# WangChangqi98/CSS

Hardware: NVIDIA B200
Metric: contrastive_path_pixels_per_sec (higher is better)
Workload: dtype f32

## Files before the change

### css_b200/csrc/css_grad.cu

```cuda
#include "css_common.cuh"

#define GSL_ELEMS 8192
#define GSL_THREADS 256
#define GSL_BATCH 24
#define GSL_PF_ANCH 3
#define GSL_LIST_MAX 6144

__device__ __forceinline__ void slab_apply(float* __restrict__ slab, const float* __restrict__ grad_anchor, float go, int a, int s, int hw,
                                           int r0, int q0, int m0, int q1, int m1) {
    const int d_min = q0 + (s < m0), d_max = q1 - (s > m1);
    const float* ga = grad_anchor + (size_t)a * CSS_D;
    for (int d = d_min; d <= d_max; d += 4) {
        float g[4];
#pragma unroll
        for (int u = 0; u < 4; ++u) g[u] = (d + u <= d_max) ? __ldg(ga + d + u) : 0.f;
#pragma unroll
        for (int u = 0; u < 4; ++u)
            if (d + u <= d_max) atomicAdd(&slab[(d + u) * hw + s - r0], go * g[u]);
    }
}

__global__ void __launch_bounds__(GSL_THREADS, 4) grad_slab_kernel(const float* __restrict__ grad_out, const int32_t* __restrict__ anchor_px,
                                                                   const float* __restrict__ grad_anchor, int n_anchor, int hw,
                                                                   int list_cap, float* __restrict__ grad_rep) {
    css_pdl_enter();
    extern __shared__ __align__(16) float slab[];
    __shared__ int s_cnt;
    int* list_a = reinterpret_cast<int*>(slab + GSL_ELEMS);
    int* list_s = list_a + list_cap;
    const int b = blockIdx.y;
    const int img = CSS_D * hw;
    const int px_lo = b * hw, px_hi = px_lo + hw;
    if (threadIdx.x == 0) s_cnt = 0;
    __syncthreads();
    for (int a0 = 0; a0 < n_anchor; a0 += GSL_THREADS * GSL_BATCH) {
        int px[GSL_BATCH];
#pragma unroll
        for (int i = 0; i < GSL_BATCH; ++i) {
            const int a = a0 + i * GSL_THREADS + threadIdx.x;
            px[i] = a < n_anchor ? __ldg(anchor_px + a) : -1;
        }
#pragma unroll
        for (int i = 0; i < GSL_BATCH; ++i) {
            if (px[i] >= px_lo && px[i] < px_hi) {
                const int pos = atomicAdd(&s_cnt, 1);
                if (pos < list_cap) {
                    list_a[pos] = a0 + i * GSL_THREADS + threadIdx.x;
                    list_s[pos] = px[i] - px_lo;
                }
            }
        }
    }
    __syncthreads();
    const int cnt = s_cnt;
    const float go = __ldg(grad_out);
    float4* slab4 = reinterpret_cast<float4*>(slab);
    float* out_img = grad_rep + (size_t)b * img;
    const int n_slabs = (img + GSL_ELEMS - 1) / GSL_ELEMS;
    for (int i = threadIdx.x; i < GSL_ELEMS / 4; i += GSL_THREADS) slab4[i] = make_float4(0.f, 0.f, 0.f, 0.f);
    __syncthreads();
    if (cnt <= GSL_THREADS * GSL_PF_ANCH && cnt <= list_cap && 2 * hw >= GSL_ELEMS) {
        float pv[GSL_PF_ANCH][2];
        int po[GSL_PF_ANCH][2];
        auto gather = [&](int j) {
            const int r0 = j * GSL_ELEMS, r1 = min(r0 + GSL_ELEMS, img);
            const int q0 = r0 / hw, m0 = r0 - q0 * hw, q1 = (r1 - 1) / hw, m1 = (r1 - 1) - q1 * hw;
#pragma unroll
            for (int u = 0; u < GSL_PF_ANCH; ++u) {
                const int t = threadIdx.x + u * GSL_THREADS;
                po[u][0] = po[u][1] = -1;
                if (t < cnt) {
                    const int a = list_a[t], sp = list_s[t];
                    const int d_min = q0 + (sp < m0), d_max = q1 - (sp > m1);
                    const float* ga = grad_anchor + (size_t)a * CSS_D;
#pragma unroll
                    for (int c = 0; c < 2; ++c) {
                        if (d_min + c <= d_max) {
                            pv[u][c] = __ldg(ga + d_min + c);
                            po[u][c] = (d_min + c) * hw + sp - r0;
                        }
                    }
                }
            }
        };
        int j = blockIdx.x;
        if (j < n_slabs) gather(j);
        for (; j < n_slabs; j += gridDim.x) {
#pragma unroll
            for (int u = 0; u < GSL_PF_ANCH; ++u)
#pragma unroll
                for (int c = 0; c < 2; ++c)
                    if (po[u][c] >= 0) atomicAdd(&slab[po[u][c]], go * pv[u][c]);
            __syncthreads();
            const int r0 = j * GSL_ELEMS, r1 = min(r0 + GSL_ELEMS, img);
            if (j + (int)gridDim.x < n_slabs) gather(j + gridDim.x);
            float4* out4 = reinterpret_cast<float4*>(out_img + r0);
            const int n4 = (r1 - r0) >> 2;
            for (int i = threadIdx.x; i < GSL_ELEMS / 4; i += GSL_THREADS) {
                if (i < n4) __stcs(out4 + i, slab4[i]);
                slab4[i] = make_float4(0.f, 0.f, 0.f, 0.f);
            }
            __syncthreads();
        }
        return;
    }
    for (int j = blockIdx.x; j < n_slabs; j += gridDim.x) {
        const int r0 = j * GSL_ELEMS, r1 = min(r0 + GSL_ELEMS, img);
        const int q0 = r0 / hw, m0 = r0 - q0 * hw, q1 = (r1 - 1) / hw, m1 = (r1 - 1) - q1 * hw;
        if (cnt <= list_cap) {
            for (int t = threadIdx.x; t < cnt; t += GSL_THREADS) slab_apply(slab, grad_anchor, go, list_a[t], list_s[t], hw, r0, q0, m0, q1, m1);
        } else {
            for (int a = threadIdx.x; a < n_anchor; a += GSL_THREADS) {
                const int px = __ldg(anchor_px + a);
                if (px >= px_lo && px < px_hi) slab_apply(slab, grad_anchor, go, a, px - px_lo, hw, r0, q0, m0, q1, m1);
            }
        }
        __syncthreads();
        float4* out4 = reinterpret_cast<float4*>(out_img + r0);
        const int n4 = (r1 - r0) >> 2;
        for (int i = threadIdx.x; i < GSL_ELEMS / 4; i += GSL_THREADS) {
            if (i < n4) __stcs(out4 + i, slab4[i]);
            slab4[i] = make_float4(0.f, 0.f, 0.f, 0.f);
        }
        __syncthreads();
    }
}

#define GS_PER_BLOCK 8
__global__ void __launch_bounds__(CSS_D) grad_scatter_kernel(const float* __restrict__ grad_out, const int32_t* __restrict__ anchor_px,
                                                             const float* __restrict__ grad_anchor, int n_anchor, int hw,
                                                             float* __restrict__ grad_rep) {
    css_pdl_enter();
    const int base = blockIdx.x * GS_PER_BLOCK;
    int px[GS_PER_BLOCK];
    float g[GS_PER_BLOCK];
#pragma unroll
    for (int i = 0; i < GS_PER_BLOCK; ++i) px[i] = (base + i < n_anchor) ? __ldg(anchor_px + base + i) : -1;
    const float go = __ldg(grad_out);
#pragma unroll
    for (int i = 0; i < GS_PER_BLOCK; ++i)
        g[i] = (px[i] >= 0) ? ldg_stream(grad_anchor + (size_t)(base + i) * CSS_D + threadIdx.x) : 0.f;
#pragma unroll
    for (int i = 0; i < GS_PER_BLOCK; ++i) {
        if (px[i] < 0) continue;
        const int b = px[i] / hw, s = px[i] - b * hw;
        atomicAdd(grad_rep + ((size_t)b * CSS_D + threadIdx.x) * hw + s, go * g[i]);
    }
}

#define GSL_MAX_ANCHORS 32768

extern "C" int css_grad_scatter(const float* grad_out, const int32_t* anchor_px, const float* grad_anchor, int n_anchor, int B2,
                                int D, int h, int w, float* grad_rep, void* stream) {
    CSS_CHECK_ARG(grad_out && anchor_px && grad_anchor && grad_rep, CSS_E_ARG, "css_grad_scatter: null pointer");
    CSS_CHECK_ARG(n_anchor > 0 && B2 > 0 && h > 0 && w > 0, CSS_E_ARG, "css_grad_scatter: non-positive size");
    CSS_CHECK_ARG(D == CSS_D, CSS_E_DIM, "css_grad_scatter: D must be %d", CSS_D);
    cudaStream_t st = (cudaStream_t)stream;
    const long long total = (long long)B2 * D * h * w;
    if (n_anchor <= GSL_MAX_ANCHORS && ((uintptr_t)grad_rep & 15) == 0 && B2 <= 65535 && (long long)D * h * w < (1ll << 30)) {
        int list_cap = 4 * ((n_anchor + B2 - 1) / B2);
        if (list_cap < 1024) list_cap = 1024;
        if (list_cap > n_anchor) list_cap = n_anchor;
        if (list_cap > GSL_LIST_MAX) list_cap = GSL_LIST_MAX;
        const int smem = GSL_ELEMS * (int)sizeof(float) + 2 * list_cap * (int)sizeof(int);
        cudaError_t e = cudaFuncSetAttribute(grad_slab_kernel, cudaFuncAttributeMaxDynamicSharedMemorySize, smem);
        if (e != cudaSuccess) { css_set_error("css_grad_scatter: cudaFuncSetAttribute: %s", cudaGetErrorString(e)); return (int)e; }
        const int n_slabs = (int)(((long long)D * h * w + GSL_ELEMS - 1) / GSL_ELEMS);
        int per_sm = (227 * 1024) / (smem + 1024);
        if (per_sm > 4) per_sm = 4;
        int G = per_sm * css_sm_count() / B2;
        if (G > n_slabs) G = n_slabs;
        if (G < 1) G = 1;
        css_launch(grad_slab_kernel, dim3(dim3(G, B2)), dim3(GSL_THREADS), (size_t)(smem), (cudaStream_t)(st), grad_out, anchor_px, grad_anchor, n_anchor, h * w, list_cap, grad_rep);
        CSS_CHECK_LAUNCH("css_grad_scatter", 1);
        return 0;
    }
    cudaError_t e = cudaMemsetAsync(grad_rep, 0, sizeof(float) * (size_t)total, st);
    if (e != cudaSuccess) { css_set_error("css_grad_scatter: memset: %s", cudaGetErrorString(e)); return (int)e; }
    css_launch(grad_scatter_kernel, dim3((n_anchor + GS_PER_BLOCK - 1) / GS_PER_BLOCK), dim3(CSS_D), (size_t)(0), (cudaStream_t)(st), grad_out, anchor_px, grad_anchor, n_anchor, h * w,
                                                                                      grad_rep);
    CSS_CHECK_LAUNCH("css_grad_scatter", 1);
    return 0;
}


__global__ void __launch_bounds__(CSS_D) grad_rows_kernel(const float* __restrict__ grad_out, const int32_t* __restrict__ anchor_px,
                                                          const float* __restrict__ grad_anchor, int n_anchor, float* __restrict__ grad_rows) {
    css_pdl_enter();
    const int base = blockIdx.x * GS_PER_BLOCK;
    int px[GS_PER_BLOCK];
    float g[GS_PER_BLOCK];
#pragma unroll
    for (int i = 0; i < GS_PER_BLOCK; ++i) px[i] = (base + i < n_anchor) ? __ldg(anchor_px + base + i) : -1;
    const float go = __ldg(grad_out);
#pragma unroll
    for (int i = 0; i < GS_PER_BLOCK; ++i)
        g[i] = (px[i] >= 0) ? ldg_stream(grad_anchor + (size_t)(base + i) * CSS_D + threadIdx.x) : 0.f;
#pragma unroll
    for (int i = 0; i < GS_PER_BLOCK; ++i)
        if (px[i] >= 0) atomicAdd(grad_rows + (size_t)px[i] * CSS_D + threadIdx.x, go * g[i]);
}

extern "C" int css_grad_scatter_nhwc(const float* grad_out, const int32_t* anchor_px, const float* grad_anchor, int n_anchor, int B2, int D,
                                     int h, int w, float* grad_rows, void* stream) {
    CSS_CHECK_ARG(grad_out && anchor_px && grad_anchor && grad_rows, CSS_E_ARG, "css_grad_scatter_nhwc: null pointer");
    CSS_CHECK_ARG(n_anchor > 0 && B2 > 0 && h > 0 && w > 0, CSS_E_ARG, "css_grad_scatter_nhwc: non-positive size");
    CSS_CHECK_ARG(D == CSS_D, CSS_E_DIM, "css_grad_scatter_nhwc: D must be %d", CSS_D);
    cudaStream_t st = (cudaStream_t)stream;
    cudaError_t e = cudaMemsetAsync(grad_rows, 0, sizeof(float) * (size_t)B2 * D * h * w, st);
    if (e != cudaSuccess) { css_set_error("css_grad_scatter_nhwc: memset: %s", cudaGetErrorString(e)); return (int)e; }
    css_launch(grad_rows_kernel, dim3((n_anchor + GS_PER_BLOCK - 1) / GS_PER_BLOCK), dim3(CSS_D), (size_t)0, st, grad_out, anchor_px, grad_anchor, n_anchor,
               grad_rows);
    CSS_CHECK_LAUNCH("css_grad_scatter_nhwc", 1);
    return 0;
}
```

Measured before the change: 228.0 million.

## Double-buffer slab and write out with TMA bulk async stores

The slab accumulator is split into two shared-memory buffers, and each finished slab is written to global memory by a single-thread cp.async.bulk store with an L2 evict-first hint. This replaces the per-thread streaming store-and-clear loop, so the bulk write of one slab can overlap the atomics into the next. The slab size is halved to 4096 elements, and the prefetch and non-prefetch paths are merged into one loop. It also adds DIAG macros that can skip work, though they are off by default. The costs are a proxy fence and a wait_group on every iteration.

```diff
diff --git a/css_b200/csrc/css_grad.cu b/css_b200/csrc/css_grad.cu
--- a/css_b200/csrc/css_grad.cu
+++ b/css_b200/csrc/css_grad.cu
@@ -1,6 +1,17 @@
 #include "css_common.cuh"
 
-#define GSL_ELEMS 8192
+#ifndef GSL_ELEMS
+#define GSL_ELEMS 4096
+#endif
+#ifndef GSL_DIAG
+#define GSL_DIAG 0
+#endif
+#ifndef GSL_MINB
+#define GSL_MINB 4
+#endif
+#ifndef GSL_NBUF
+#define GSL_NBUF 2
+#endif
 #define GSL_THREADS 256
 #define GSL_BATCH 24
 #define GSL_PF_ANCH 3
@@ -20,20 +31,27 @@
     }
 }
 
-__global__ void __launch_bounds__(GSL_THREADS, 4) grad_slab_kernel(const float* __restrict__ grad_out, const int32_t* __restrict__ anchor_px,
+__device__ __forceinline__ void bulk_store(float* dst, const float* src, int bytes, uint64_t policy) {
+    const uint32_t s = (uint32_t)__cvta_generic_to_shared(src);
+    asm volatile("cp.async.bulk.global.shared::cta.bulk_group.L2::cache_hint [%0], [%1], %2, %3;" ::"l"(dst), "r"(s), "r"(bytes), "l"(policy)
+                 : "memory");
+    asm volatile("cp.async.bulk.commit_group;" ::: "memory");
+}
+
+__global__ void __launch_bounds__(GSL_THREADS, GSL_MINB) grad_slab_kernel(const float* __restrict__ grad_out, const int32_t* __restrict__ anchor_px,
                                                                    const float* __restrict__ grad_anchor, int n_anchor, int hw,
                                                                    int list_cap, float* __restrict__ grad_rep) {
     css_pdl_enter();
-    extern __shared__ __align__(16) float slab[];
+    extern __shared__ __align__(128) float slab[];
     __shared__ int s_cnt;
-    int* list_a = reinterpret_cast<int*>(slab + GSL_ELEMS);
+    int* list_a = reinterpret_cast<int*>(slab + GSL_NBUF * GSL_ELEMS);
     int* list_s = list_a + list_cap;
     const int b = blockIdx.y;
     const int img = CSS_D * hw;
     const int px_lo = b * hw, px_hi = px_lo + hw;
     if (threadIdx.x == 0) s_cnt = 0;
     __syncthreads();
-    for (int a0 = 0; a0 < n_anchor; a0 += GSL_THREADS * GSL_BATCH) {
+    for (int a0 = 0; a0 < (GSL_DIAG == 1 || GSL_DIAG == 2 ? 0 : n_anchor); a0 += GSL_THREADS * GSL_BATCH) {
         int px[GSL_BATCH];
 #pragma unroll
         for (int i = 0; i < GSL_BATCH; ++i) {
@@ -54,76 +72,66 @@
     __syncthreads();
     const int cnt = s_cnt;
     const float go = __ldg(grad_out);
-    float4* slab4 = reinterpret_cast<float4*>(slab);
     float* out_img = grad_rep + (size_t)b * img;
     const int n_slabs = (img + GSL_ELEMS - 1) / GSL_ELEMS;
-    for (int i = threadIdx.x; i < GSL_ELEMS / 4; i += GSL_THREADS) slab4[i] = make_float4(0.f, 0.f, 0.f, 0.f);
-    __syncthreads();
-    if (cnt <= GSL_THREADS * GSL_PF_ANCH && cnt <= list_cap && 2 * hw >= GSL_ELEMS) {
-        float pv[GSL_PF_ANCH][2];
-        int po[GSL_PF_ANCH][2];
-        auto gather = [&](int j) {
-            const int r0 = j * GSL_ELEMS, r1 = min(r0 + GSL_ELEMS, img);
-            const int q0 = r0 / hw, m0 = r0 - q0 * hw, q1 = (r1 - 1) / hw, m1 = (r1 - 1) - q1 * hw;
-#pragma unroll
-            for (int u = 0; u < GSL_PF_ANCH; ++u) {
-                const int t = threadIdx.x + u * GSL_THREADS;
-                po[u][0] = po[u][1] = -1;
-                if (t < cnt) {
-                    const int a = list_a[t], sp = list_s[t];
-                    const int d_min = q0 + (sp < m0), d_max = q1 - (sp > m1);
-                    const float* ga = grad_anchor + (size_t)a * CSS_D;
-#pragma unroll
-                    for (int c = 0; c < 2; ++c) {
-                        if (d_min + c <= d_max) {
-                            pv[u][c] = __ldg(ga + d_min + c);
-                            po[u][c] = (d_min + c) * hw + sp - r0;
-                        }
+    uint64_t policy = 0;
+    if (threadIdx.x == 0) asm volatile("createpolicy.fractional.L2::evict_first.b64 %0, 1.0;" : "=l"(policy));
+    const bool pf = cnt <= GSL_THREADS * GSL_PF_ANCH && cnt <= list_cap && 2 * hw >= GSL_ELEMS;
+    float pv[GSL_PF_ANCH][2];
+    int po[GSL_PF_ANCH][2];
+    auto gather = [&](int j) {
+        const int r0 = j * GSL_ELEMS, r1 = min(r0 + GSL_ELEMS, img);
+        const int q0 = r0 / hw, m0 = r0 - q0 * hw, q1 = (r1 - 1) / hw, m1 = (r1 - 1) - q1 * hw;
+#pragma unroll
+        for (int u = 0; u < GSL_PF_ANCH; ++u) {
+            const int t = threadIdx.x + u * GSL_THREADS;
+            po[u][0] = po[u][1] = -1;
+            if (t < cnt) {
+                const int a = list_a[t], sp = list_s[t];
+                const int d_min = q0 + (sp < m0), d_max = q1 - (sp > m1);
+                const float* ga = grad_anchor + (size_t)a * CSS_D;
+#pragma unroll
+                for (int c = 0; c < 2; ++c) {
+                    if (d_min + c <= d_max) {
+                        pv[u][c] = __ldg(ga + d_min + c);
+                        po[u][c] = (d_min + c) * hw + sp - r0;
                     }
                 }
             }
-        };
-        int j = blockIdx.x;
-        if (j < n_slabs) gather(j);
-        for (; j < n_slabs; j += gridDim.x) {
+        }
+    };
+    if (pf && blockIdx.x < n_slabs) gather(blockIdx.x);
+    int k = 0;
+    for (int j = blockIdx.x; j < n_slabs; j += gridDim.x, ++k) {
+        float* buf = slab + (k % GSL_NBUF) * GSL_ELEMS;
+        float4* buf4 = reinterpret_cast<float4*>(buf);
+        if (GSL_DIAG != 2) for (int i = threadIdx.x; i < GSL_ELEMS / 4; i += GSL_THREADS) buf4[i] = make_float4(0.f, 0.f, 0.f, 0.f);
+        __syncthreads();
+        const int r0 = j * GSL_ELEMS, r1 = min(r0 + GSL_ELEMS, img);
+        if (pf) {
 #pragma unroll
             for (int u = 0; u < GSL_PF_ANCH; ++u)
 #pragma unroll
                 for (int c = 0; c < 2; ++c)
-                    if (po[u][c] >= 0) atomicAdd(&slab[po[u][c]], go * pv[u][c]);
-            __syncthreads();
-            const int r0 = j * GSL_ELEMS, r1 = min(r0 + GSL_ELEMS, img);
+                    if (po[u][c] >= 0) atomicAdd(&buf[po[u][c]], go * pv[u][c]);
             if (j + (int)gridDim.x < n_slabs) gather(j + gridDim.x);
-            float4* out4 = reinterpret_cast<float4*>(out_img + r0);
-            const int n4 = (r1 - r0) >> 2;
-            for (int i = threadIdx.x; i < GSL_ELEMS / 4; i += GSL_THREADS) {
-                if (i < n4) __stcs(out4 + i, slab4[i]);
-                slab4[i] = make_float4(0.f, 0.f, 0.f, 0.f);
+        } else {
+            const int q0 = r0 / hw, m0 = r0 - q0 * hw, q1 = (r1 - 1) / hw, m1 = (r1 - 1) - q1 * hw;
+            if (cnt <= list_cap) {
+                for (int t = threadIdx.x; t < cnt; t += GSL_THREADS) slab_apply(buf, grad_anchor, go, list_a[t], list_s[t], hw, r0, q0, m0, q1, m1);
+            } else {
+                for (int a = threadIdx.x; a < n_anchor; a += GSL_THREADS) {
+                    const int px = __ldg(anchor_px + a);
+                    if (px >= px_lo && px < px_hi) slab_apply(buf, grad_anchor, go, a, px - px_lo, hw, r0, q0, m0, q1, m1);
+                }
             }
-            __syncthreads();
-        }
-        return;
-    }
-    for (int j = blockIdx.x; j < n_slabs; j += gridDim.x) {
-        const int r0 = j * GSL_ELEMS, r1 = min(r0 + GSL_ELEMS, img);
-        const int q0 = r0 / hw, m0 = r0 - q0 * hw, q1 = (r1 - 1) / hw, m1 = (r1 - 1) - q1 * hw;
-        if (cnt <= list_cap) {
-            for (int t = threadIdx.x; t < cnt; t += GSL_THREADS) slab_apply(slab, grad_anchor, go, list_a[t], list_s[t], hw, r0, q0, m0, q1, m1);
-        } else {
-            for (int a = threadIdx.x; a < n_anchor; a += GSL_THREADS) {
-                const int px = __ldg(anchor_px + a);
-                if (px >= px_lo && px < px_hi) slab_apply(slab, grad_anchor, go, a, px - px_lo, hw, r0, q0, m0, q1, m1);
-            }
-        }
+        }
+        asm volatile("fence.proxy.async.shared::cta;" ::: "memory");
+        if (threadIdx.x == 0) asm volatile("cp.async.bulk.wait_group.read %0;" ::"n"(GSL_NBUF - 2) : "memory");
         __syncthreads();
-        float4* out4 = reinterpret_cast<float4*>(out_img + r0);
-        const int n4 = (r1 - r0) >> 2;
-        for (int i = threadIdx.x; i < GSL_ELEMS / 4; i += GSL_THREADS) {
-            if (i < n4) __stcs(out4 + i, slab4[i]);
-            slab4[i] = make_float4(0.f, 0.f, 0.f, 0.f);
-        }
-        __syncthreads();
-    }
+        if (threadIdx.x == 0) bulk_store(out_img + r0, buf, (r1 - r0) * (int)sizeof(float), policy);
+    }
+    if (threadIdx.x == 0) { if (GSL_DIAG == 3) asm volatile("cp.async.bulk.wait_group.read 0;" ::: "memory"); else asm volatile("cp.async.bulk.wait_group 0;" ::: "memory"); }
 }
 
 #define GS_PER_BLOCK 8
@@ -162,12 +170,12 @@
         if (list_cap < 1024) list_cap = 1024;
         if (list_cap > n_anchor) list_cap = n_anchor;
         if (list_cap > GSL_LIST_MAX) list_cap = GSL_LIST_MAX;
-        const int smem = GSL_ELEMS * (int)sizeof(float) + 2 * list_cap * (int)sizeof(int);
+        const int smem = GSL_NBUF * GSL_ELEMS * (int)sizeof(float) + 2 * list_cap * (int)sizeof(int);
         cudaError_t e = cudaFuncSetAttribute(grad_slab_kernel, cudaFuncAttributeMaxDynamicSharedMemorySize, smem);
         if (e != cudaSuccess) { css_set_error("css_grad_scatter: cudaFuncSetAttribute: %s", cudaGetErrorString(e)); return (int)e; }
         const int n_slabs = (int)(((long long)D * h * w + GSL_ELEMS - 1) / GSL_ELEMS);
         int per_sm = (227 * 1024) / (smem + 1024);
-        if (per_sm > 4) per_sm = 4;
+        if (per_sm > GSL_MINB) per_sm = GSL_MINB;
         int G = per_sm * css_sm_count() / B2;
         if (G > n_slabs) G = n_slabs;
         if (G < 1) G = 1;
```

Result: no change. 229.1 million, median of 6 (+0.5%).
